# theteamatx/x-edr-trajectory-planning

Hardware: AMD Instinct MI355X
Metric: time-optimal path timings/s (7-DOF, 2000 s-samples), 1/2/4/8 MI355X + %HBM roofline (higher is better)
Workload: dtype f64

## Files before the change

### include/tpamd.h

```cpp
#ifndef TPAMD_H_
#define TPAMD_H_

#include <stddef.h>
#include <stdint.h>

#ifdef __cplusplus
extern "C" {
#endif

#define TPAMD_VERSION 200

#define TPAMD_E_INVALID_ARGUMENT (-1)
#define TPAMD_E_HIP (-2)
#define TPAMD_E_UNSUPPORTED (-3)
#define TPAMD_E_NO_DEVICE (-4)
#define TPAMD_E_STALE (-5)

#define TPAMD_PATH_OK 0
#define TPAMD_PATH_INFEASIBLE_BOUNDS 2
#define TPAMD_PATH_S_RANGE 3
#define TPAMD_PATH_SD_START_NEGATIVE 4
#define TPAMD_PATH_LOWER_GE_UPPER 5
#define TPAMD_PATH_TOO_FEW_SAMPLES 6
#define TPAMD_PATH_NO_CONNECTION 7
#define TPAMD_PATH_NAN_SD2 8
#define TPAMD_PATH_NONZERO_END 9
#define TPAMD_PATH_CRIT_INDEX_ZERO 10
#define TPAMD_PATH_NO_WAYPOINTS 11

typedef struct tpamd_engine tpamd_engine;

int tpamd_engine_create(int device_ordinal, tpamd_engine **out);
void tpamd_engine_destroy(tpamd_engine *engine);
int tpamd_version(void);
const char *tpamd_error_string(int code);
int tpamd_device_count(void);
int tpamd_engine_reserve(tpamd_engine *engine, int num_paths, int num_samples,
                         int num_rows);
int tpamd_engine_set_pipelining(tpamd_engine *engine, int mode);
int tpamd_engine_fence(tpamd_engine *engine, void *hip_stream);
size_t tpamd_engine_workspace_bytes(const tpamd_engine *engine);

typedef struct tpamd_joint_batch {
// ... 727 lines not shown
```

### x-edr-trajectory-planning_amd/csrc/tpamd_capi.hip

```cpp
#include "../../include/tpamd.h"

#include <hip/hip_runtime.h>

#include <algorithm>
#include <cmath>
#include <cstdio>
#include <cstdlib>
#include <cstring>
#include <mutex>
#include <new>
#include <vector>

#include "tpamd_kernels.h"
#include "tpamd_launch.h"
#include "tpamd_planner_set.h"
#include "tpamd_readout.h"
#include "tpamd_rescale.h"
#include "tpamd_buffer.h"
#include "tpamd_stop.h"
#include "tpamd_switch.h"
#include "tpamd_fit.h"
#include "tpamd_retarget.h"
#include "tpamd_pose_fit.h"
#include "tpamd_joint_fit.h"
// ... 488 lines not shown
    case TPAMD_E_INVALID_ARGUMENT: return "invalid argument";
    case TPAMD_E_HIP: return "HIP runtime error";
    case TPAMD_E_UNSUPPORTED: return "unsupported size";
    case TPAMD_E_NO_DEVICE: return "no HIP device";
    case TPAMD_E_STALE: return "engine state belongs to a different solve";
    case TPAMD_PATH_INFEASIBLE_BOUNDS: return "infeasible bounds: no upper > lower at a sample";
    case TPAMD_PATH_S_RANGE: return "s_start must be < s_end";
    case TPAMD_PATH_SD_START_NEGATIVE: return "sd_start must be >= 0";
    case TPAMD_PATH_LOWER_GE_UPPER: return "constraints must satisfy lower < upper";
    case TPAMD_PATH_TOO_FEW_SAMPLES: return "need at least 2 samples";
    case TPAMD_PATH_NO_CONNECTION: return "could not connect from critical point to initial trajectory portion";
    case TPAMD_PATH_NAN_SD2: return "no solution found (NaN in sd2)";
    case TPAMD_PATH_NONZERO_END: return "non-zero terminal velocity";
    case TPAMD_PATH_CRIT_INDEX_ZERO: return "critical point search degenerated to index 0";
    case TPAMD_PATH_NO_WAYPOINTS: return "path without waypoints";
    default: return "unknown";
  }
}

int tpamd_device_count(void) {
  int count = 0;
  if (hipGetDeviceCount(&count) != hipSuccess || count < 0) return 0;
  return count;
}

void tpamd_shard_bounds(int num_paths, int num_shards, int32_t *begin) {
  if (!begin || num_shards <= 0) return;
  const int total = num_paths > 0 ? num_paths : 0;
  const int base = total / num_shards, rem = total % num_shards;
  for (int r = 0; r <= num_shards; r++) begin[r] = r * base + (r < rem ? r : rem);
// ... 5261 lines not shown
```

### x-edr-trajectory-planning_amd/csrc/tpamd_sweep_joint.h

```cpp
#pragma once

#include <type_traits>

#include "tpamd_kernels.h"

namespace tpamd {

__device__ __forceinline__ double uniform_f64(double v) {
  const int lo = __builtin_amdgcn_readfirstlane(__double2loint(v));
  const int hi = __builtin_amdgcn_readfirstlane(__double2hiint(v));
  return __hiloint2double(hi, lo);
}
__device__ __forceinline__ double readlane_f64(double v, int lane) {
  const int lo = __builtin_amdgcn_readlane(__double2loint(v), lane);
  const int hi = __builtin_amdgcn_readlane(__double2hiint(v), lane);
  return __hiloint2double(hi, lo);
}
__device__ __forceinline__ int uniform_i32(int v) { return __builtin_amdgcn_readfirstlane(v); }
__device__ __forceinline__ int lds_word(const int *p) {
  return *(const volatile __attribute__((address_space(3))) int *)p;
}

template <int CTRL>
__device__ __forceinline__ double dpp_f64(double v) {
// ... 121 lines not shown
#define TPAMD_ACC(slot, var)
#endif
#else
#define TPAMD_T0(var)
#define TPAMD_ACC(slot, var)
#define TPAMD_T0C(var)
#define TPAMD_ACCC(slot, var)
#define TPAMD_CNT(slot)
#define TPAMD_ADD(slot, v)
#define TPAMD_CNTX(slot)
#endif

#ifndef TPAMD_CHAIN_GUESS
#define TPAMD_CHAIN_GUESS 0
#endif
constexpr int kTileSamples = 32;
template <int D>
struct TileCfg {
  static constexpr int kSamples = (D > 8) ? 16 : kTileSamples;
};

typedef double f64x2 __attribute__((ext_vector_type(2)));

template <int K>
struct RegPack {
  f64x2 v;
  RegPack<K - 1> rest;
  template <int LIMIT>
  __device__ __forceinline__ void load(const f64x2 *src, int c) {
    if (c < LIMIT) v = src[c];
    rest.template load<LIMIT>(src, c + 64);
  }
  template <int LIMIT>
  __device__ __forceinline__ void store(f64x2 *dst, int c) const {
    if (c < LIMIT) dst[c] = v;
    rest.template store<LIMIT>(dst, c + 64);
  }
};
template <>
struct RegPack<0> {
  template <int LIMIT> __device__ __forceinline__ void load(const f64x2 *, int) {}
  template <int LIMIT> __device__ __forceinline__ void store(f64x2 *, int) const {}
};

template <int D>
struct JointLayout {
  static constexpr int PARTS = (D <= 7) ? 4 : ((D <= 16) ? 2 : 1);
  static constexpr int RPL = (D + PARTS - 1) / PARTS;
  static constexpr int kCandLanes = 2 * D * PARTS;
  static constexpr int kRows16 = (kCandLanes + 15) / 16;
  static_assert(kCandLanes <= 64, "candidate lanes must fit one wave");
  static constexpr int kChain = 16;
  static constexpr int GRP = 64 / kChain;
  static constexpr int CPL = (2 * D + GRP - 1) / GRP;
  static constexpr int VPL = (D + GRP - 1) / GRP;
  static constexpr unsigned long long kPart0 =
      (GRP == 4) ? 0x1111111111111111ull : ((GRP == 2) ? 0x5555555555555555ull : ~0ull);
// ... 19 lines not shown
  mutable long long diagx[kDiagExt];
#endif
  int N, lane;
  double ds, two_ds;
  double *sd2;
  double *tiles;
  const uint8_t *typel;
  double *sdd_g;
  const double *m_g;
  const double *rec;
  int tag0, tag1;
  double *qd_g, *qdd_g;
  const double *aml;
  uint32_t *dirty;
  int end_idx;
  double lim;
  double chk_hi[L::RPL];
  double vel_hi;
  double vel_lo;
  int vel_mode;
  double ex_hi[E ? E : 1];
  int own_off;
  int chk_off[L::RPL];
  int vel_off;
  double row_lo, row_hi;
  double v_lim[L::CPL];
  int v_off[L::CPL];
  double vv_hi[L::VPL];
  double va_hi[L::VPL];
  int vv_off[L::VPL];

  struct Rows {
    f64x2 own;
    f64x2 chk[L::RPL];
    f64x2 vel;
  };

  static __device__ __forceinline__ void wave_lds_sync() {
    __builtin_amdgcn_fence(__ATOMIC_ACQ_REL, "wavefront");
    __builtin_amdgcn_wave_barrier();
  }

  struct Prefetch {
    RegPack<kChunksPerLane> r;
    double m;
    int tag;
  };
  __device__ __forceinline__ void issue_tile_loads(int t, Prefetch &pf) const {
    const f64x2 *src = reinterpret_cast<const f64x2 *>(rec + (size_t)t * kTile * R);
    pf.r.template load<kChunks>(src, lane);
    pf.m = m_g[min(t * kTile + (lane & (kTile - 1)), N - 1)];
    pf.tag = t;
  }
  __device__ __forceinline__ void store_tile(int slot, const Prefetch &pf) const {
    f64x2 *dst = reinterpret_cast<f64x2 *>(tiles + (size_t)slot * kTile * R);
    pf.r.template store<kChunks>(dst, lane);
    wave_lds_sync();
    if (lane < kTile) {
      const int i = min(pf.tag * kTile + lane, N - 1);
      f64x2 mt;
      mt.x = pf.m;
// ... 50 lines not shown
    if (QDD) {
      const double v2 = v * v;
      double acc = pr.x * a + pr.y * v2;
      if (acc < -amx) acc = -amx;
      if (acc > amx) acc = amx;
      qdd_g[o] = acc;
    }
  }
  __device__ __forceinline__ void emit_value(int i, int d, f64x2 pr, double v, double a,
                                             double amx) const {
    const size_t o = (size_t)i * D + d;
    if (qd_g) emit_pair<true, false>(o, pr, v, a, amx);
    if (qdd_g) emit_pair<false, true>(o, pr, v, a, amx);
  }
  __device__ __forceinline__ int emit_range(int lo, int hi, int wv, int nwv, const int *stop = nullptr,
                                            int stop_value = 0) const {
    if (qd_g != nullptr && qdd_g != nullptr) return emit_trips<true, true>(lo, hi, wv, nwv, stop, stop_value);
    if (qd_g != nullptr) return emit_trips<true, false>(lo, hi, wv, nwv, stop, stop_value);
    if (qdd_g != nullptr) return emit_trips<false, true>(lo, hi, wv, nwv, stop, stop_value);
    return hi + 1;
  }
  template <bool QD, bool QDD>
  __device__ __forceinline__ int emit_trips(int lo, int hi, int wv, int nwv, const int *stop,
                                            int stop_value) const {
    int s0 = lo + 64 * wv;
    if (hi < lo || s0 > hi) return hi + 1;
    if (stop != nullptr && uniform_i32(lds_word(stop)) == stop_value) return s0;
    const int step = 64 * nwv;
    const f64x2 *rec2 = reinterpret_cast<const f64x2 *>(rec);
    constexpr int G = (D <= 8) ? D : 5;
    constexpr int NG = (D + G - 1) / G;
    int ln = lane;
    asm volatile("" : "+v"(ln));
    int se0[D];
#pragma unroll
    for (int p = 0; p < D; p++) se0[p] = (64 * p + ln) / D;
    auto joint_of = [&](int p) { return 64 * p + ln - se0[p] * D; };
    f64x2 pr[2][G];
    double s2l[2], al[2];
    auto issue_sample = [&](int t0, int h) {
      const int mine = min(t0 + lane, hi);
      s2l[h] = sd2[mine];
// ... 33 lines not shown
          for (int g = 0; g < G; g++) {
            const int p = k * G + g;
            if (p >= D) continue;
            const int se = min(se0[p], last), dd = joint_of(p);
            const int src = se << 2;
            const double v = __hiloint2double(__builtin_amdgcn_ds_bpermute(src, __double2hiint(vl)),
                                              __builtin_amdgcn_ds_bpermute(src, __double2loint(vl)));
            const double a = __hiloint2double(__builtin_amdgcn_ds_bpermute(src, __double2hiint(al[h])),
                                              __builtin_amdgcn_ds_bpermute(src, __double2loint(al[h])));
            emit_pair<QD, QDD>((size_t)(s0 + se) * D + dd, pr[set][g], v, a, aml[dd]);
            if (p & 1) __builtin_amdgcn_sched_barrier(0);
          }
        }
        s0 = nxt;
        if (s0 > hi) return hi + 1;
        if (stop != nullptr && uniform_i32(lds_word(stop)) == stop_value) return s0;
      }
    }
  }
  __device__ __forceinline__ void mark_dirty(int i) const {
    if (lane == 0) atomicOr(&dirty[i >> 5], 1u << (i & 31));
  }

  template <bool MAX>
  __device__ __forceinline__ double find_sdd(const Rows &r, double s2, int &win) const {
    constexpr double kSentinel = MAX ? -DBL_MAX : DBL_MAX;
    bool vel_bad;
    if (E == 0) {
      const double vv = (r.vel.x * r.vel.x) * s2;
      vel_bad = (vv + kTiny < 0.0) | (vv - kTiny > vel_hi);
    } else {
// ... 125 lines not shown
  }

  struct Carry {
    int idx;
    double cur;
    double m_i;
    double m_n;
    double nxt;
    int t_i, t_n;
    int win;
  };
  static constexpr int kContinue = -2;

  template <bool FWD>
  __device__ __forceinline__ int extremal_step(Carry &c, const Rows &use, Rows &stage, Prefetch &pf,
                                               int idx_start, bool &pair_signal, bool &pair_wait) {
    constexpr int dir = FWD ? 1 : -1;
#define TPAMD_PAIR_SIGNAL()                                   \
  do {                                                        \
    if (pair_signal) {                                        \
      __threadfence_block();                                  \
      __syncthreads();                                        \
      pair_signal = false;                                    \
    }                                                         \
  } while (0)
#define TPAMD_PAIR_WAIT()                                     \
  do {                                                        \
    if (FWD && pair_wait) {                                   \
      __syncthreads();                                        \
      pair_wait = false;                                      \
    }                                                         \
  } while (0)
    const int idx = c.idx;
    const int nidx = idx + dir;
    const bool more = FWD ? (nidx < N - 2) : (nidx > 1);
    if (((nidx + dir) & (kTile - 1)) == (FWD ? 0 : kTile - 1))
      ensure_tile(nidx + dir, dir, pf);
    load_rows(nidx, stage);
    double m_nn;
    int t_nn;
    load_mt(nidx + dir, m_nn, t_nn);
    const double nxt_nn = sd2[nidx + dir];
    const double cur = c.cur, m_i = c.m_i, m_n = c.m_n, nxt = c.nxt;
    const bool on_boundary = is_tiny(cur - m_i);
    double sd2tmp, sddtmp;
    if (on_boundary && (c.t_i & kBndTrajectory) && (c.t_n & kBndTrajectory)) {
// ... 10 lines not shown
    if (!isnan(nxt) && (nxt < sd2tmp)) {
      TPAMD_PAIR_WAIT();
      sdd_at_intersection(idx);
      TPAMD_PAIR_SIGNAL();
      return FWD ? N - 1 : 0;
    }
    if (sd2tmp > m_n) {
      const double sdd_bound = FWD ? 0.5 * (m_n - cur) / ds : 0.5 * (cur - m_n) / ds;
      const bool deriv_invalid = !derivs_valid(idx, sdd_bound, FWD ? m_i : cur);
      const bool type_invalid = c.t_n & (FWD ? kBndSink : kBndSource);
      const bool stop = FWD ? (type_invalid || deriv_invalid)
                            : ((type_invalid || deriv_invalid) && !(idx_start != (N - 1)));
      if (stop) {
        end_idx = idx;
        TPAMD_PAIR_SIGNAL();
        TPAMD_PAIR_WAIT();
        return idx;
      }
      sd2tmp = m_n;
      sddtmp = sdd_bound;
      c.win = -1;
    }
    if (sd2tmp < 0) {
      TPAMD_PAIR_WAIT();
      c.win = -1;
      sd2tmp = 0.0;
      if (FWD) {
        if (idx <= 1) sddtmp = 0.0; else sddtmp = -sd2[idx - 1] / ds;
      } else {
        if (idx < N - 1) sddtmp = sd2[idx + 1] / ds; else sddtmp = 0.0;
      }
    }
    TPAMD_PAIR_WAIT();
    put_sd2(nidx, sd2tmp);
    put_sdd(idx, sddtmp);
    if (!more) end_idx = nidx;
    TPAMD_PAIR_SIGNAL();
    if (!more) return FWD ? N - 1 : 0;
    c.idx = nidx;
    c.cur = sd2tmp;
    c.m_i = m_n;
    c.t_i = c.t_n;
    c.m_n = uniform_f64(m_nn);
    c.t_n = uniform_i32(t_nn);
    c.nxt = uniform_f64(nxt_nn);
    return kContinue;
#undef TPAMD_PAIR_SIGNAL
#undef TPAMD_PAIR_WAIT
  }

// ... 8 lines not shown
    const int tj = max(j, 0) / kTile, tjn = max(jn, 0) / kTile;
    const bool resident = (tj == tag0 || tj == tag1) && (tjn == tag0 || tjn == tag1);
    if (in_loop && j >= 0 && j < N && resident) {
      const f64x2 mt_j = record(j)[kMt], mt_n = record(jn)[kMt];
      m_j = mt_j.x;
      m_jn = mt_n.x;
      const double nxt = sd2[jn];
      elig = (__double2loint(mt_j.y) & kBndTrajectory) && (__double2loint(mt_n.y) & kBndTrajectory) &&
             !(!isnan(nxt) && (nxt < m_jn)) && !(m_jn < 0);
    }
    const unsigned long long mask = __ballot(elig);
    const int L = (~mask == 0ull) ? 64 : (__ffsll((long long)~mask) - 1);
    if (L == 0) return 0;
    const double cur_k = (lane == 0) ? c.cur : m_j;
    const double sddv = FWD ? 0.5 * (m_jn - cur_k) / ds : 0.5 * (cur_k - m_jn) / ds;
    if (lane < L) {
      sd2[j + dir] = m_jn;
      sdd_g[j] = sddv;
    }
    wave_lds_sync();
    c.idx += dir * L;
    c.cur = readlane_f64(m_jn, L - 1);
    return L;
  }

  template <bool FWD>
  __device__ __forceinline__ int follow_chain(Carry &c, Prefetch &pf, int &next_win, bool &curve) {
    constexpr int dir = FWD ? 1 : -1;
    constexpr int K = L::kChain;
    next_win = -1;
    curve = false;
    const int wl = c.win;
    const int r = (wl / L::PARTS) >> 1;
// ... 96 lines not shown
    const int idx = c.idx, nidx = idx + dir;
    const bool more = FWD ? (nidx < N - 2) : (nidx > 1);
    const double cur = c.cur, m_n = c.m_n;
    const double sdd_bound = FWD ? 0.5 * (m_n - cur) / ds : 0.5 * (cur - m_n) / ds;
    const bool deriv_invalid = !derivs_valid(idx, sdd_bound, FWD ? c.m_i : cur);
    const bool type_invalid = c.t_n & (FWD ? kBndSink : kBndSource);
    const bool stop = FWD ? (type_invalid || deriv_invalid)
                          : ((type_invalid || deriv_invalid) && !(idx_start != (N - 1)));
    if (stop) {
      end_idx = idx;
      return idx;
    }
    double sd2tmp = m_n, sddtmp = sdd_bound;
    c.win = -1;
    if (sd2tmp < 0) {
      sd2tmp = 0.0;
      if (FWD) {
        if (idx <= 1) sddtmp = 0.0; else sddtmp = -sd2[idx - 1] / ds;
      } else {
        if (idx < N - 1) sddtmp = sd2[idx + 1] / ds; else sddtmp = 0.0;
      }
    }
    put_sd2(nidx, sd2tmp);
    put_sdd(idx, sddtmp);
    if (!more) {
      end_idx = nidx;
      return FWD ? N - 1 : 0;
    }
    c.idx = nidx;
    c.cur = sd2tmp;
// ... 15 lines not shown
    load_mt(idx, m0, t0);
    load_mt(idx + dir, m1, t1);
    c.m_i = uniform_f64(m0); c.m_n = uniform_f64(m1);
    c.t_i = uniform_i32(t0); c.t_n = uniform_i32(t1);
    c.nxt = uniform_f64(sd2[idx + dir]);
    c.win = -1;
    TPAMD_ACC(26, ti_);
  }

  template <bool FWD>
  __device__ __forceinline__ int add_extremal(int idx_start, Prefetch &pf, bool pair_signal = false,
                                              bool wait_pair = false) {
#define TPAMD_PAIR_SIGNAL()                                   \
  do {                                                        \
    if (pair_signal) {                                        \
      __threadfence_block();                                  \
      __syncthreads();                                        \
      pair_signal = false;                                    \
    }                                                         \
  } while (0)
    if (FWD ? !(idx_start < N - 2) : !(idx_start > 1)) {
      end_idx = idx_start;
      TPAMD_PAIR_SIGNAL();
      if (wait_pair) __syncthreads();
      return FWD ? N - 1 : 0;
    }
    Rows rows_a, rows_b;
    Carry c;
    init_carry<FWD>(idx_start, c, rows_a, pf, true);
    if (wait_pair && is_tiny(c.cur - c.m_i) && (c.t_i & kBndTrajectory) && (c.t_n & kBndTrajectory)) {
      __syncthreads();
      wait_pair = false;
    }
    bool trust = true;
    int last_win = -1;
    for (;;) {
#define TPAMD_TRY_FOLLOW()                                                                   \
  if (is_tiny(c.cur - c.m_i) && (c.t_i & kBndTrajectory) && (c.t_n & kBndTrajectory)) {      \
    TPAMD_T0(tfb_);                                                                          \
    const int run = uniform_i32(follow_boundary<FWD>(c));                                    \
    TPAMD_ACC(25, tfb_);                                                                     \
    if (run > 0) {                                                                           \
      TPAMD_CNT(8);                                                                          \
      TPAMD_PAIR_SIGNAL();                                                                   \
      if (FWD ? !(c.idx < N - 2) : !(c.idx > 1)) {                                           \
        end_idx = c.idx;                                                                     \
        return FWD ? N - 1 : 0;                                                              \
      }                                                                                      \
// ... 25 lines not shown
      total = 1;          \
    }                                                                                        \
    if (total > 0) {                                                                         \
      if (FWD ? !(c.idx < N - 2) : !(c.idx > 1)) {                                           \
        end_idx = c.idx;                                                                     \
        return FWD ? N - 1 : 0;                                                              \
      }                                                                                      \
      init_carry<FWD>(c.idx, c, rows_a, pf, false);                                          \
      continue;                                                                              \
    }                                                                                        \
  } else {                                                                                   \
    last_win = c.win;                                                                        \
  }
      TPAMD_TRY_FOLLOW();
      TPAMD_T0(ts1_);
      int r = extremal_step<FWD>(c, rows_a, rows_b, pf, idx_start, pair_signal, wait_pair);
      TPAMD_ACC(24, ts1_);
      if (r != kContinue) return r;
      TPAMD_TRY_CHAIN();
      if (is_tiny(c.cur - c.m_i) && (c.t_i & kBndTrajectory) && (c.t_n & kBndTrajectory)) {
        load_rows(c.idx, rows_a);
        continue;
      }
      TPAMD_T0(ts2_);
      r = extremal_step<FWD>(c, rows_b, rows_a, pf, idx_start, pair_signal, wait_pair);
      TPAMD_ACC(24, ts2_);
      if (r != kContinue) return r;
      TPAMD_TRY_CHAIN();
    }
#undef TPAMD_TRY_CHAIN
#undef TPAMD_TRY_FOLLOW
#undef TPAMD_PAIR_SIGNAL
  }

  __device__ __forceinline__ int next_critical_point(int idx_lo, int idx_hi, int zlast) const {
    int c0 = -1;
    for (int base = idx_lo + 1; base <= idx_hi && c0 < 0; base += 256) {
      uint8_t ty[4];
#pragma unroll
      for (int u = 0; u < 4; u++) ty[u] = typel[min(base + 64 * u + lane, N - 1)];
// ... 493 lines not shown
      }
      if (P.count + 64 > kRefitCap) P.template flush<true>(diag);
      P.append(refit, j, m, m_next);
    }
  }
  P.template flush<true>(diag);
  __threadfence_block();
  __syncthreads();
  TPAMD_ACCC(22, tp0);
}

template <int D, int E = 0>
struct SweepLds {
  static constexpr int R = 2 * D + E + 2;
  static constexpr int kRingDoubles = 2 * 2 * TileCfg<D>::kSamples * R;
  __host__ __device__ static constexpr int n2(int N) { return (N + 1) & ~1; }
  __host__ __device__ static constexpr int words(int N) { return ((N + 31) / 32 + 1) & ~1; }
  __host__ __device__ static constexpr int type_bytes(int N) { return ((N + 15) / 16) * 16; }
  __host__ __device__ static constexpr size_t bytes(int N) {
    return (size_t)n2(N) * 8 + (size_t)kRingDoubles * 8 + type_bytes(N) + 64 +
           2 * (size_t)words(N) * 4 + 16 * 8 + 32;
  }
};
template <int D, int E = 0>
__host__ __device__ inline size_t sweep_joint_lds_bytes(int N) {
  return SweepLds<D, E>::bytes(N);
}

constexpr int kSweepWavesPerEu = 2;
constexpr int kSweepWavesPerEuWide = 1;
template <int D, int E = 0>
__global__ void __launch_bounds__(128)
__attribute__((amdgpu_waves_per_eu((D > 8) ? kSweepWavesPerEuWide : kSweepWavesPerEu,
                                   (D > 8) ? kSweepWavesPerEuWide : kSweepWavesPerEu)))
k_sweep_joint(int stride, int max_loops, JointSource src, Workspace ws, double *t_out, double *s_out,
// ... 17 lines not shown
      if (dtmax_out) dtmax_out[b] = -1.0;
    }
    return;
  }
  JS S;
  S.N = N; S.lane = lane;
  S.ds = ws.ds[b];
  S.two_ds = 2.0 * S.ds;
  S.sd2 = lds;
  double *ring = lds + LL::n2(N);
  S.tiles = ring + (size_t)w * 2 * JS::kTile * JS::R;
  uint8_t *typel = reinterpret_cast<uint8_t *>(ring + LL::kRingDoubles);
  S.typel = typel;
  int *xchg = reinterpret_cast<int *>(typel + LL::type_bytes(N));
  const int nw = LL::words(N);
  uint32_t *dirty = reinterpret_cast<uint32_t *>(xchg + 16);
  uint32_t *zero = dirty + nw;
  double *aml = reinterpret_cast<double *>(zero + nw);
  double *red = aml + 16;
  S.dirty = dirty;
  S.aml = aml;
  S.sdd_g = sdd_out + pb;
  S.m_g = ws.m + pb;
  S.rec = src.q12 + pb * JS::R;
  S.qd_g = qd_out ? qd_out + pb * D : nullptr;
  S.qdd_g = qdd_out ? qdd_out + pb * D : nullptr;
  S.end_idx = 0;
  S.tag0 = -1; S.tag1 = -1;
  double *sd2 = S.sd2;
  const double sd_start = ws.sd_start[b];
#ifdef TPAMD_DIAG
  long long(&diag)[32] = S.diag;
  long long(&diagx)[kDiagExt] = S.diagx;
  for (int k = 0; k < 32; k++) diag[k] = 0;
  for (int k = 0; k < kDiagExt; k++) diagx[k] = 0;
  volatile long long *fw_stamp = reinterpret_cast<volatile long long *>(red + 2);
#define TPAMD_DIAG_PTR S.diag
#else
#define TPAMD_DIAG_PTR nullptr
#endif
  boundary_passes_for_path<D, E>(src, ws, b, N, stride, tid, reinterpret_cast<uint8_t *>(sd2),
                           reinterpret_cast<uint8_t *>(sd2) + LL::type_bytes(N),
                           reinterpret_cast<char *>(ring), typel, (ws.keep_boundary & 1) != 0,
                           TPAMD_DIAG_PTR);
  constexpr int C = 2 * D + E;
  const double *lim_lo = src.lim + (size_t)b * 2 * C, *lim_hi = lim_lo + C;
  {
    typedef JointLayout<D> L;
    const double kInf = __longlong_as_double(0x7ff0000000000000LL);
    const bool is_cand = lane < L::kCandLanes;
    const int c = is_cand ? lane / L::PARTS : 0;
// ... 45 lines not shown
      S.vv_off[i] = has ? row : 0;
      S.vv_hi[i] = has ? lim_hi[D + row] : kInf;
      S.va_hi[i] = has ? lim_hi[row] : kInf;
    }
  }

  for (int i = tid; i < N; i += 128) {
    sd2[i] = qnan();
    S.sdd_g[i] = qnan();
  }
  for (int i = tid; i < 2 * nw; i += 128) dirty[i] = 0u;
  if (tid < D) aml[tid] = ws.amax ? ws.amax[(size_t)b * D + tid] : 0.0;
  __syncthreads();
  if (tid == 0) {
    xchg[2] = 0;
    xchg[6] = 0;
    sd2[0] = sd_start * sd_start;
    sd2[N - 1] = 0;
  }
  __syncthreads();

  int status = 0;
  int iforw_lo = 0, iback_hi = N - 1, iback_lo, iforw_hi, icrit, icrit_lo, icrit_hi;
  typename JS::Prefetch pf;
  pf.tag = -1;
  TPAMD_T0C(t_all);
  int emitted_hi = 0, upper_lo = N;
  bool first_pair_in_order = false;
  if (w == 0) {
    const int r = S.template add_extremal<false>(iback_hi, pf);
    if (lane == 0) { xchg[0] = r; xchg[7] = S.end_idx; }
// ... 36 lines not shown
    __syncthreads();
  }
  iback_lo = uniform_i32(xchg[0]);
  iforw_hi = uniform_i32(xchg[1]);
  TPAMD_ACCC(9, t_all);
  icrit_hi = iback_lo;
  if ((iforw_hi < icrit_hi) && ((icrit_hi < N - 2) && (icrit_hi >= 2))) {
    if (w == 0) S.put_sd2(icrit_hi, qnan());
    icrit_hi++;
    iback_lo++;
  }
  icrit_lo = iforw_hi;
  const int zlast = uniform_i32(S.last_flagged_below(icrit_hi));
  const double *m_g = ws.m + pb;
  if (max_loops <= 0) max_loops = max(100, 10 * N);
  double *crit_m = reinterpret_cast<double *>(xchg + 10);
  auto post_next_critical_point = [&](int lo) {
    TPAMD_T0(t0);
    int ic = uniform_i32(S.next_critical_point(lo, icrit_hi, zlast));
    TPAMD_ACC(2, t0);
#if defined(TPAMD_DIAG) && !defined(TPAMD_DIAG_LIGHT)
    {
      TPAMD_T0(tl_);
      if (ic != S.next_critical_point_literal(lo, icrit_hi)) TPAMD_CNT(7);
      TPAMD_ACC(18, tl_);
    }
#endif
    if (ic < 0 || ic >= N) ic = (int)(0.5 * (lo + icrit_hi));
    const double mc = m_g[min(max(ic, 0), N - 1)], mp = m_g[min(max(ic - 1, 0), N - 1)];
    if (ic >= 1) {
      const int ts = ic / JS::kTile;
      const int tag = (ts & 1) ? S.tag1 : S.tag0;
      if (tag != ts && pf.tag != ts) S.issue_tile_loads(ts, pf);
    }
    if (lane == 0) {
      xchg[9] = ic;
      crit_m[0] = mc;
      crit_m[1] = mp;
    }
  };
  __syncthreads();
  if (w == 1 && iforw_hi < icrit_hi) post_next_critical_point(icrit_lo);
  __threadfence_block();
  __syncthreads();
  for (int loop = 0; loop < max_loops; loop++) {
    if (iforw_hi >= icrit_hi) break;
    TPAMD_CNT(11);
#ifdef TPAMD_DIAG
    int bw_case = 2;
    long long bw_left = 0;
#endif
    icrit = uniform_i32(xchg[9]);
    const double m_c = uniform_f64(crit_m[0]), m_p = uniform_f64(crit_m[1]);
    if (w == 0 && icrit >= 1) {
      const int ts = (icrit - 1) / JS::kTile;
      const int tag = (ts & 1) ? S.tag1 : S.tag0;
      if (tag != ts && pf.tag != ts) S.issue_tile_loads(ts, pf);
    }
    if (icrit > 0 && icrit < N - 1 && w == 0) S.put_sd2(icrit, m_c);
    if (icrit < 1) { status = 10; break; }
    if (m_p <= m_c) {
      iback_hi = icrit - 1;
      if (w == 0) S.put_sd2(icrit - 1, m_p);
    } else {
      iback_hi = icrit;
    }
    iforw_lo = icrit;
    __syncthreads();
    {
      TPAMD_T0C(t0);
      if (w == 0) {
        const int r = S.template add_extremal<false>(iback_hi, pf, true);
        if (lane == 0) xchg[0] = r;
#ifdef TPAMD_DIAG
        const bool fw_was_done = lds_word(xchg + 6) == loop + 1;
#endif
        TPAMD_T0C(te);
        emitted_hi = uniform_i32(S.emit_range(max(min(S.end_idx - 1, emitted_hi), 0), icrit - 1,
                                              0, 1, xchg + 6, loop + 1));
        TPAMD_ACCC(12, te);
#ifdef TPAMD_DIAG
        bw_case = fw_was_done ? 0 : (lds_word(xchg + 6) == loop + 1) ? 1 : 2;
        bw_left = tpamd_stamp();
#endif
      } else {
        const int r = S.template add_extremal<true>(iforw_lo, pf, false, true);
#ifdef TPAMD_DIAG
        { const long long t = tpamd_stamp(); if (lane == 0) fw_stamp[0] = t; }
#endif
        if (lane == 0) {
          xchg[1] = r;
          *reinterpret_cast<volatile int *>(xchg + 6) = loop + 1;
        }
        if (r < icrit_hi) post_next_critical_point(r);
#ifdef TPAMD_DIAG
        { const long long t = tpamd_stamp(); if (lane == 0) fw_stamp[1] = t; }
#endif
      }
      TPAMD_ACCC(0, t0);
    }
    {
      TPAMD_T0C(t0);
      __threadfence_block();
#ifdef TPAMD_DIAG
      const long long fenced = tpamd_stamp();
#endif
      __syncthreads();
      TPAMD_ACCC(1, t0);
#ifdef TPAMD_DIAG
      if (w == 0) {
        const long long fw_done = fw_stamp[0], fw_at_c = fw_stamp[1];
        const long long fw_wait = (fenced > fw_at_c) ? fenced - fw_at_c : 0;
        diagx[0] += bw_case == 0;
        diagx[1] += bw_case == 1;
        diagx[2] += bw_case == 2;
        diagx[7] += fenced - t0;
        if (bw_case == 1) {
          diagx[3] += bw_left - fw_done;
          diagx[4] += fenced - t0;
          diagx[5] += fw_wait;
        } else if (bw_case == 0) {
          diagx[6] += fw_wait;
        }
      }
#endif
    }
    iback_lo = uniform_i32(xchg[0]);
    iforw_hi = uniform_i32(xchg[1]);
    if (iback_lo > icrit_lo) { status = 7; break; }
    icrit_lo = iforw_hi;
  }
  TPAMD_ACCC(5, t_all);
  if (lane == 0) {
    if (w == 0) { xchg[4] = emitted_hi; xchg[5] = upper_lo; }
    else xchg[3] = S.end_idx;
  }
  __threadfence_block();
  __syncthreads();

  TPAMD_T0C(t_tail);
  const double ds = S.ds;
  double *sdd = S.sdd_g;
  {
    int has_nan = 0;
    if (status == 0)
      for (int idx = tid; idx < N; idx += 128)
        if (isnan(sd2[idx])) has_nan = 1;
    if (has_nan) xchg[2] = 1;
    __syncthreads();
    if (status == 0 && xchg[2] != 0) status = 8;
  }
  if (status == 0) {
    for (int base = 0; base < N; base += 512) {
// ... 250 lines not shown
```

### x-edr-trajectory-planning_amd/engine.py

```python
import ctypes as C
import os

import numpy as np

from . import abi as _abi
from .abi import (
    ABI_SYMBOLS, DIAG_SO, HIPCC_FLAGS, MULTI_SO, PLAN_DEVICE_INFO_FIELDS, PLAN_RESOURCE_EXHAUSTED,
    PLANNER_CHECK_DTYPE, PLANNER_STATE_INFO_DTYPE, PLANNER_SUMMARY_DTYPE, REFINE_NO_SLOT, REFINE_NOTHING,
    REFINE_TOO_LONG, SWEEP_INSTANCES, TpamdError, _CartesianBatch, _CartesianInputs, _CheckOutputs,
    _FastestStopArgs, _JointBatch, _JointInputs, _PathOutputs, _PlanDeviceInfo, _PlannerCheck, _PlannerSetConfig,
    _RefineOptions, _RefineOutputs, _ResampleArgs, _RowsBatch, _RowsInputs, _Solution, _StopTrajectoryArgs,
    _WaypointBatch, _WaypointFitOutputs, _WaypointInputs, _ptr)

_SO = os.environ.get("TPAMD_LIBRARY") or os.path.join(_abi._CSRC, "libtpamd.so")

PATH_STATUS = {
    0: "ok", 2: "infeasible_bounds", 3: "s_range", 4: "sd_start_negative",
    5: "lower_ge_upper", 6: "too_few_samples", 7: "no_connection", 8: "nan_sd2",
    9: "nonzero_end", 10: "crit_index_zero", 11: "no_waypoints",
}

KERNEL_SWEEP = 4

_CARTESIAN_INPUT_KEYS = _CartesianInputs._keys_


def build_library(force=False, verbose=False, extra_flags=(), output=None):
    global _SO
    if output is not None:
        _SO = output
    return _abi._compile(_SO, extra_flags, force, verbose)


def build_multi_library(force=False, verbose=False):
# ... 1526 lines not shown
```

Measured before the change: 2.161 million.

## Decouple forward and backward sweep waves with an LDS work queue

The per-loop __syncthreads lockstep between the forward wave and the backward wave is replaced by a 4-entry LDS ring queue. The forward wave finds critical points, posts them, and keeps integrating ahead while the backward wave consumes entries and emits outputs. The first overlapping write is handed off through a compare-exchange in LDS, so neither wave has to block on a workgroup barrier. This is meant to remove barrier stalls and let the two directions overlap across loops. In exchange it adds spin-polling with s_sleep, a bounded-wait error status, and ordering logic that is subtle and could race.

```diff
diff --git a/include/tpamd.h b/include/tpamd.h
--- a/include/tpamd.h
+++ b/include/tpamd.h
@@ -27,6 +27,7 @@
 #define TPAMD_PATH_NONZERO_END 9
 #define TPAMD_PATH_CRIT_INDEX_ZERO 10
 #define TPAMD_PATH_NO_WAYPOINTS 11
+#define TPAMD_PATH_SWEEP_POLL_EXPIRED 12
 
 typedef struct tpamd_engine tpamd_engine;
 
diff --git a/x-edr-trajectory-planning_amd/csrc/tpamd_capi.hip b/x-edr-trajectory-planning_amd/csrc/tpamd_capi.hip
--- a/x-edr-trajectory-planning_amd/csrc/tpamd_capi.hip
+++ b/x-edr-trajectory-planning_amd/csrc/tpamd_capi.hip
@@ -526,6 +526,7 @@
     case TPAMD_PATH_NONZERO_END: return "non-zero terminal velocity";
     case TPAMD_PATH_CRIT_INDEX_ZERO: return "critical point search degenerated to index 0";
     case TPAMD_PATH_NO_WAYPOINTS: return "path without waypoints";
+    case TPAMD_PATH_SWEEP_POLL_EXPIRED: return "internal error: a bounded wait inside the sweep kernel ran out";
     default: return "unknown";
   }
 }
diff --git a/x-edr-trajectory-planning_amd/csrc/tpamd_sweep_joint.h b/x-edr-trajectory-planning_amd/csrc/tpamd_sweep_joint.h
--- a/x-edr-trajectory-planning_amd/csrc/tpamd_sweep_joint.h
+++ b/x-edr-trajectory-planning_amd/csrc/tpamd_sweep_joint.h
@@ -159,6 +159,20 @@
 #ifndef TPAMD_CHAIN_GUESS
 #define TPAMD_CHAIN_GUESS 0
 #endif
+constexpr int kQRing = 4;
+constexpr int kQEntryWords = 16;
+constexpr int kQPosted = 6;
+constexpr int kQDone1 = 9;
+constexpr int kQAbort = 10;
+constexpr int kQStatus = 11;
+constexpr int kQPollErr = 12;
+constexpr int kQeState = 0, kQeCrit = 1, kQeBackHi = 2, kQeCritLo = 3, kQeKind = 4;
+constexpr int kQeDeferred = 8;
+constexpr int kQKindLoop = 0, kQKindEnd = 1, kQKindCritZero = 2;
+constexpr int kQPollBound = 1 << 22;
+constexpr int kStatusSweepPoll = 12;
+static_assert(kQPosted < 16 && kQPollErr < 16 && kQeDeferred + 4 <= kQEntryWords, "loop queue layout");
+
 constexpr int kTileSamples = 32;
 template <int D>
 struct TileCfg {
@@ -181,11 +195,16 @@
     if (c < LIMIT) dst[c] = v;
     rest.template store<LIMIT>(dst, c + 64);
   }
+  __device__ __forceinline__ void drop() {
+    v = f64x2{0.0, 0.0};
+    rest.drop();
+  }
 };
 template <>
 struct RegPack<0> {
   template <int LIMIT> __device__ __forceinline__ void load(const f64x2 *, int) {}
   template <int LIMIT> __device__ __forceinline__ void store(f64x2 *, int) const {}
+  __device__ __forceinline__ void drop() {}
 };
 
 template <int D>
@@ -235,6 +254,10 @@
   const double *aml;
   uint32_t *dirty;
   int end_idx;
+  int *qc, *qe;
+  int qn;
+  int pair_mode;
+  bool fw_first;
   double lim;
   double chk_hi[L::RPL];
   double vel_hi;
@@ -262,10 +285,97 @@
     __builtin_amdgcn_wave_barrier();
   }
 
+  static __device__ __forceinline__ void lds_store(int *p, int v) {
+    *(volatile __attribute__((address_space(3))) int *)p = v;
+  }
+  template <int CAUSE>
+  __device__ __forceinline__ bool q_wait(int word, int value) const {
+    if (uniform_i32(lds_word(qc + word)) >= value) return true;
+#ifdef TPAMD_DIAG
+    const long long tw_ = tpamd_stamp();
+#endif
+    bool ok = false;
+    for (int n = 0;; n++) {
+      __builtin_amdgcn_s_sleep(1);
+      if (uniform_i32(lds_word(qc + word)) >= value) { ok = true; break; }
+      if (uniform_i32(lds_word(qc + kQAbort)) != 0) break;
+      if (n >= kQPollBound) {
+        if (lane == 0) { lds_store(qc + kQPollErr, 1); lds_store(qc + kQAbort, 1); }
+        break;
+      }
+    }
+#ifdef TPAMD_DIAG
+    diagx[CAUSE] += tpamd_stamp() - tw_;
+    diagx[CAUSE + 9] += 1;
+#endif
+    return ok;
+  }
+  __device__ __forceinline__ void pair_release() {
+    __threadfence_block();
+    int old = 0;
+    if (lane == 0) {
+      int expected = 4 * qn + 1;
+      __hip_atomic_compare_exchange_strong(qe + kQeState, &expected, 4 * qn + 2, __ATOMIC_RELAXED,
+                                           __ATOMIC_RELAXED, __HIP_MEMORY_SCOPE_WORKGROUP);
+      old = expected;
+    }
+    fw_first = uniform_i32(old) == 4 * qn + 3;
+    __threadfence_block();
+#ifdef TPAMD_DIAG
+    diagx[5] += fw_first;
+    diagx[6] += !fw_first;
+#endif
+    if (fw_first && lane == 0) {
+      const int c = lds_word(qe + kQeCrit);
+      const volatile __attribute__((address_space(3))) double *pd =
+          (const volatile __attribute__((address_space(3))) double *)(qe + kQeDeferred);
+      sd2[c + 1] = pd[0];
+      sdd_g[c] = pd[1];
+    }
+    __threadfence_block();
+    if (lane == 0) lds_store(qc + kQDone1, qn + 1);
+  }
+  __device__ __forceinline__ bool pair_defer(double v, double a) {
+    if (uniform_i32(lds_word(qc + kQDone1)) > qn) { pair_mode = 0; return false; }
+    int old = 0;
+    if (lane == 0) {
+      volatile __attribute__((address_space(3))) double *pd =
+          (volatile __attribute__((address_space(3))) double *)(qe + kQeDeferred);
+      pd[0] = v;
+      pd[1] = a;
+    }
+    __threadfence_block();
+    if (lane == 0) {
+      int expected = 4 * qn + 1;
+      __hip_atomic_compare_exchange_strong(qe + kQeState, &expected, 4 * qn + 3, __ATOMIC_RELAXED,
+                                           __ATOMIC_RELAXED, __HIP_MEMORY_SCOPE_WORKGROUP);
+      old = expected;
+    }
+    old = uniform_i32(old);
+    if (old == 4 * qn + 1) {
+      TPAMD_CNTX(5);
+      pair_mode = 2;
+      return true;
+    }
+    __threadfence_block();
+    pair_mode = 0;
+    return false;
+  }
+  template <int CAUSE>
+  __device__ __forceinline__ void pair_settle() {
+    q_wait<CAUSE>(kQDone1, qn + 1);
+    pair_mode = 0;
+  }
+
   struct Prefetch {
     RegPack<kChunksPerLane> r;
     double m;
     int tag;
+    __device__ __forceinline__ void drop() {
+      r.drop();
+      m = 0.0;
+      tag = -1;
+    }
   };
   __device__ __forceinline__ void issue_tile_loads(int t, Prefetch &pf) const {
     const f64x2 *src = reinterpret_cast<const f64x2 *>(rec + (size_t)t * kTile * R);
@@ -346,18 +456,18 @@
     if (qdd_g) emit_pair<false, true>(o, pr, v, a, amx);
   }
   __device__ __forceinline__ int emit_range(int lo, int hi, int wv, int nwv, const int *stop = nullptr,
-                                            int stop_value = 0) const {
-    if (qd_g != nullptr && qdd_g != nullptr) return emit_trips<true, true>(lo, hi, wv, nwv, stop, stop_value);
-    if (qd_g != nullptr) return emit_trips<true, false>(lo, hi, wv, nwv, stop, stop_value);
-    if (qdd_g != nullptr) return emit_trips<false, true>(lo, hi, wv, nwv, stop, stop_value);
+                                            int go_value = 0) const {
+    if (qd_g != nullptr && qdd_g != nullptr) return emit_trips<true, true>(lo, hi, wv, nwv, stop, go_value);
+    if (qd_g != nullptr) return emit_trips<true, false>(lo, hi, wv, nwv, stop, go_value);
+    if (qdd_g != nullptr) return emit_trips<false, true>(lo, hi, wv, nwv, stop, go_value);
     return hi + 1;
   }
   template <bool QD, bool QDD>
   __device__ __forceinline__ int emit_trips(int lo, int hi, int wv, int nwv, const int *stop,
-                                            int stop_value) const {
+                                            int go_value) const {
     int s0 = lo + 64 * wv;
     if (hi < lo || s0 > hi) return hi + 1;
-    if (stop != nullptr && uniform_i32(lds_word(stop)) == stop_value) return s0;
+    if (stop != nullptr && uniform_i32(lds_word(stop)) != go_value) return s0;
     const int step = 64 * nwv;
     const f64x2 *rec2 = reinterpret_cast<const f64x2 *>(rec);
     constexpr int G = (D <= 8) ? D : 5;
@@ -421,7 +531,7 @@
         }
         s0 = nxt;
         if (s0 > hi) return hi + 1;
-        if (stop != nullptr && uniform_i32(lds_word(stop)) == stop_value) return s0;
+        if (stop != nullptr && uniform_i32(lds_word(stop)) != go_value) return s0;
       }
     }
   }
@@ -577,22 +687,18 @@
 
   template <bool FWD>
   __device__ __forceinline__ int extremal_step(Carry &c, const Rows &use, Rows &stage, Prefetch &pf,
-                                               int idx_start, bool &pair_signal, bool &pair_wait) {
+                                               int idx_start, bool &pair_signal) {
     constexpr int dir = FWD ? 1 : -1;
 #define TPAMD_PAIR_SIGNAL()                                   \
   do {                                                        \
     if (pair_signal) {                                        \
-      __threadfence_block();                                  \
-      __syncthreads();                                        \
+      pair_release();                                         \
       pair_signal = false;                                    \
     }                                                         \
   } while (0)
 #define TPAMD_PAIR_WAIT()                                     \
   do {                                                        \
-    if (FWD && pair_wait) {                                   \
-      __syncthreads();                                        \
-      pair_wait = false;                                      \
-    }                                                         \
+    if (FWD && pair_mode != 0) pair_settle<0>();              \
   } while (0)
     const int idx = c.idx;
     const int nidx = idx + dir;
@@ -633,7 +739,6 @@
       if (stop) {
         end_idx = idx;
         TPAMD_PAIR_SIGNAL();
-        TPAMD_PAIR_WAIT();
         return idx;
       }
       sd2tmp = m_n;
@@ -650,9 +755,10 @@
         if (idx < N - 1) sddtmp = sd2[idx + 1] / ds; else sddtmp = 0.0;
       }
     }
-    TPAMD_PAIR_WAIT();
-    put_sd2(nidx, sd2tmp);
-    put_sdd(idx, sddtmp);
+    if (!(FWD && pair_mode == 1 && pair_defer(sd2tmp, sddtmp))) {
+      put_sd2(nidx, sd2tmp);
+      put_sdd(idx, sddtmp);
+    }
     if (!more) end_idx = nidx;
     TPAMD_PAIR_SIGNAL();
     if (!more) return FWD ? N - 1 : 0;
@@ -691,9 +797,18 @@
     if (L == 0) return 0;
     const double cur_k = (lane == 0) ? c.cur : m_j;
     const double sddv = FWD ? 0.5 * (m_jn - cur_k) / ds : 0.5 * (cur_k - m_jn) / ds;
-    if (lane < L) {
+    const bool first = FWD && pair_mode == 1;
+    if (lane < L && !(first && lane == 0)) {
       sd2[j + dir] = m_jn;
       sdd_g[j] = sddv;
+    }
+    if (first) {
+      if (pair_defer(readlane_f64(m_jn, 0), readlane_f64(sddv, 0))) {
+        TPAMD_CNTX(6);
+      } else if (lane == 0) {
+        sd2[j + dir] = m_jn;
+        sdd_g[j] = sddv;
+      }
     }
     wave_lds_sync();
     c.idx += dir * L;
@@ -820,6 +935,7 @@
     double sd2tmp = m_n, sddtmp = sdd_bound;
     c.win = -1;
     if (sd2tmp < 0) {
+      if (FWD && pair_mode != 0) pair_settle<0>();
       sd2tmp = 0.0;
       if (FWD) {
         if (idx <= 1) sddtmp = 0.0; else sddtmp = -sd2[idx - 1] / ds;
@@ -865,24 +981,19 @@
 #define TPAMD_PAIR_SIGNAL()                                   \
   do {                                                        \
     if (pair_signal) {                                        \
-      __threadfence_block();                                  \
-      __syncthreads();                                        \
+      pair_release();                                         \
       pair_signal = false;                                    \
     }                                                         \
   } while (0)
+    pair_mode = (FWD && wait_pair) ? 1 : 0;
     if (FWD ? !(idx_start < N - 2) : !(idx_start > 1)) {
       end_idx = idx_start;
       TPAMD_PAIR_SIGNAL();
-      if (wait_pair) __syncthreads();
       return FWD ? N - 1 : 0;
     }
     Rows rows_a, rows_b;
     Carry c;
     init_carry<FWD>(idx_start, c, rows_a, pf, true);
-    if (wait_pair && is_tiny(c.cur - c.m_i) && (c.t_i & kBndTrajectory) && (c.t_n & kBndTrajectory)) {
-      __syncthreads();
-      wait_pair = false;
-    }
     bool trust = true;
     int last_win = -1;
     for (;;) {
@@ -938,7 +1049,7 @@
   }
       TPAMD_TRY_FOLLOW();
       TPAMD_T0(ts1_);
-      int r = extremal_step<FWD>(c, rows_a, rows_b, pf, idx_start, pair_signal, wait_pair);
+      int r = extremal_step<FWD>(c, rows_a, rows_b, pf, idx_start, pair_signal);
       TPAMD_ACC(24, ts1_);
       if (r != kContinue) return r;
       TPAMD_TRY_CHAIN();
@@ -947,7 +1058,7 @@
         continue;
       }
       TPAMD_T0(ts2_);
-      r = extremal_step<FWD>(c, rows_b, rows_a, pf, idx_start, pair_signal, wait_pair);
+      r = extremal_step<FWD>(c, rows_b, rows_a, pf, idx_start, pair_signal);
       TPAMD_ACC(24, ts2_);
       if (r != kContinue) return r;
       TPAMD_TRY_CHAIN();
@@ -1471,11 +1582,12 @@
 struct SweepLds {
   static constexpr int R = 2 * D + E + 2;
   static constexpr int kRingDoubles = 2 * 2 * TileCfg<D>::kSamples * R;
+  static constexpr int kXchgWords = 16 + kQRing * kQEntryWords;
   __host__ __device__ static constexpr int n2(int N) { return (N + 1) & ~1; }
   __host__ __device__ static constexpr int words(int N) { return ((N + 31) / 32 + 1) & ~1; }
   __host__ __device__ static constexpr int type_bytes(int N) { return ((N + 15) / 16) * 16; }
   __host__ __device__ static constexpr size_t bytes(int N) {
-    return (size_t)n2(N) * 8 + (size_t)kRingDoubles * 8 + type_bytes(N) + 64 +
+    return (size_t)n2(N) * 8 + (size_t)kRingDoubles * 8 + type_bytes(N) + 4 * kXchgWords +
            2 * (size_t)words(N) * 4 + 16 * 8 + 32;
   }
 };
@@ -1523,7 +1635,7 @@
   S.typel = typel;
   int *xchg = reinterpret_cast<int *>(typel + LL::type_bytes(N));
   const int nw = LL::words(N);
-  uint32_t *dirty = reinterpret_cast<uint32_t *>(xchg + 16);
+  uint32_t *dirty = reinterpret_cast<uint32_t *>(xchg + LL::kXchgWords);
   uint32_t *zero = dirty + nw;
   double *aml = reinterpret_cast<double *>(zero + nw);
   double *red = aml + 16;
@@ -1536,6 +1648,8 @@
   S.qdd_g = qdd_out ? qdd_out + pb * D : nullptr;
   S.end_idx = 0;
   S.tag0 = -1; S.tag1 = -1;
+  S.qc = xchg; S.qe = xchg + 16; S.qn = 0;
+  S.pair_mode = 0; S.fw_first = false;
   double *sd2 = S.sd2;
   const double sd_start = ws.sd_start[b];
 #ifdef TPAMD_DIAG
@@ -1543,7 +1657,6 @@
   long long(&diagx)[kDiagExt] = S.diagx;
   for (int k = 0; k < 32; k++) diag[k] = 0;
   for (int k = 0; k < kDiagExt; k++) diagx[k] = 0;
-  volatile long long *fw_stamp = reinterpret_cast<volatile long long *>(red + 2);
 #define TPAMD_DIAG_PTR S.diag
 #else
 #define TPAMD_DIAG_PTR nullptr
@@ -1619,7 +1732,7 @@
   __syncthreads();
   if (tid == 0) {
     xchg[2] = 0;
-    xchg[6] = 0;
+    xchg[kQPosted] = 0; xchg[kQDone1] = 0; xchg[kQAbort] = 0; xchg[kQStatus] = 0; xchg[kQPollErr] = 0;
     sd2[0] = sd_start * sd_start;
     sd2[N - 1] = 0;
   }
@@ -1686,129 +1799,131 @@
   const int zlast = uniform_i32(S.last_flagged_below(icrit_hi));
   const double *m_g = ws.m + pb;
   if (max_loops <= 0) max_loops = max(100, 10 * N);
-  double *crit_m = reinterpret_cast<double *>(xchg + 10);
-  auto post_next_critical_point = [&](int lo) {
-    TPAMD_T0(t0);
-    int ic = uniform_i32(S.next_critical_point(lo, icrit_hi, zlast));
-    TPAMD_ACC(2, t0);
+  __syncthreads();
+  if (w == 1) {
+    int posted = 0, last_c = 0;
+    for (int loop = 0;; loop++) {
+      int kind = (loop >= max_loops || iforw_hi >= icrit_hi) ? kQKindEnd : kQKindLoop;
+      if (uniform_i32(lds_word(xchg + kQAbort)) != 0) break;
+      int ic = 0, bh = 0;
+      double mc = 0.0, mp = 0.0;
+      if (kind == kQKindLoop) {
+        TPAMD_CNT(11);
+        TPAMD_T0(t0);
+        ic = uniform_i32(S.next_critical_point(icrit_lo, icrit_hi, zlast));
+        TPAMD_ACC(2, t0);
 #if defined(TPAMD_DIAG) && !defined(TPAMD_DIAG_LIGHT)
-    {
-      TPAMD_T0(tl_);
-      if (ic != S.next_critical_point_literal(lo, icrit_hi)) TPAMD_CNT(7);
-      TPAMD_ACC(18, tl_);
-    }
+        {
+          TPAMD_T0(tl_);
+          if (ic != S.next_critical_point_literal(icrit_lo, icrit_hi)) TPAMD_CNT(7);
+          TPAMD_ACC(18, tl_);
+        }
 #endif
-    if (ic < 0 || ic >= N) ic = (int)(0.5 * (lo + icrit_hi));
-    const double mc = m_g[min(max(ic, 0), N - 1)], mp = m_g[min(max(ic - 1, 0), N - 1)];
-    if (ic >= 1) {
-      const int ts = ic / JS::kTile;
-      const int tag = (ts & 1) ? S.tag1 : S.tag0;
-      if (tag != ts && pf.tag != ts) S.issue_tile_loads(ts, pf);
+        if (ic < 0 || ic >= N) ic = (int)(0.5 * (icrit_lo + icrit_hi));
+        if (ic >= 1) {
+          const int ts = ic / JS::kTile;
+          const int tag = (ts & 1) ? S.tag1 : S.tag0;
+          if (tag != ts && pf.tag != ts) S.issue_tile_loads(ts, pf);
+        }
+        mc = uniform_f64(m_g[min(max(ic, 0), N - 1)]);
+        mp = uniform_f64(m_g[min(max(ic - 1, 0), N - 1)]);
+        if (ic < 1) kind = kQKindCritZero;
+        bh = (mp <= mc) ? ic - 1 : ic;
+      }
+      if (!S.template q_wait<2>(kQDone1, posted - (kQRing - 1))) break;
+      if (kind == kQKindLoop) {
+        if (posted > 0 && ic - 1 <= last_c + 1 && !S.template q_wait<1>(kQDone1, posted)) break;
+        if (ic < N - 1) S.put_sd2(ic, mc);
+        if (mp <= mc) S.put_sd2(ic - 1, mp);
+      }
+      int *q = xchg + 16 + kQEntryWords * (posted & (kQRing - 1));
+      if (lane == 0) {
+        q[kQeCrit] = ic;
+        q[kQeBackHi] = bh;
+        q[kQeCritLo] = icrit_lo;
+        q[kQeKind] = kind;
+      }
+      __threadfence_block();
+      if (lane == 0) {
+        JS::lds_store(q + kQeState, 4 * posted + 1);
+        JS::lds_store(xchg + kQPosted, posted + 1);
+      }
+      if (kind != kQKindLoop) break;
+      S.qe = q;
+      S.qn = posted;
+      posted++;
+      last_c = ic;
+      TPAMD_T0C(t0);
+      const int r = S.template add_extremal<true>(ic, pf, false, true);
+      TPAMD_ACCC(0, t0);
+      iforw_hi = r;
+      icrit_lo = r;
+    }
+    if (lane == 0) xchg[3] = S.end_idx;
+  } else {
+    int taken = 0;
+    for (;;) {
+      if (!S.template q_wait<0>(kQPosted, taken + 1)) break;
+      __threadfence_block();
+      int *q = xchg + 16 + kQEntryWords * (taken & (kQRing - 1));
+      const int kind = uniform_i32(lds_word(q + kQeKind));
+      if (kind != kQKindLoop) {
+        if (kind == kQKindCritZero) status = 10;
+        break;
+      }
+      TPAMD_CNT(11);
+      icrit = uniform_i32(lds_word(q + kQeCrit));
+      iback_hi = uniform_i32(lds_word(q + kQeBackHi));
+      icrit_lo = uniform_i32(lds_word(q + kQeCritLo));
+#ifdef TPAMD_DIAG
+      {
+        const int depth = uniform_i32(lds_word(xchg + kQPosted)) - taken;
+        diagx[1] += depth == 1;
+        diagx[2] += depth == 2;
+        diagx[3] += depth == 3;
+        diagx[4] += depth >= 4;
+      }
+#endif
+      {
+        const int ts = (icrit - 1) / JS::kTile;
+        const int tag = (ts & 1) ? S.tag1 : S.tag0;
+        if (tag != ts && pf.tag != ts) S.issue_tile_loads(ts, pf);
+      }
+      S.qe = q;
+      S.qn = taken;
+      TPAMD_T0C(t0);
+      const int r = S.template add_extremal<false>(iback_hi, pf, true);
+      TPAMD_ACCC(0, t0);
+      taken++;
+      iback_lo = r;
+      if (iback_lo > icrit_lo) { status = 7; break; }
+      TPAMD_T0C(te);
+      emitted_hi = uniform_i32(S.emit_range(max(min(S.end_idx - 1, emitted_hi), 0), icrit - 1,
+                                            0, 1, xchg + kQPosted, taken));
+      TPAMD_ACCC(12, te);
+      pf.drop();
     }
     if (lane == 0) {
-      xchg[9] = ic;
-      crit_m[0] = mc;
-      crit_m[1] = mp;
-    }
-  };
-  __syncthreads();
-  if (w == 1 && iforw_hi < icrit_hi) post_next_critical_point(icrit_lo);
-  __threadfence_block();
-  __syncthreads();
-  for (int loop = 0; loop < max_loops; loop++) {
-    if (iforw_hi >= icrit_hi) break;
-    TPAMD_CNT(11);
+      xchg[kQStatus] = status;
+      if (status != 0) JS::lds_store(xchg + kQAbort, 1);
+      xchg[4] = emitted_hi;
+      xchg[5] = upper_lo;
+    }
+  }
+  TPAMD_ACCC(5, t_all);
+  {
 #ifdef TPAMD_DIAG
-    int bw_case = 2;
-    long long bw_left = 0;
+    const long long tj_ = tpamd_stamp();
 #endif
-    icrit = uniform_i32(xchg[9]);
-    const double m_c = uniform_f64(crit_m[0]), m_p = uniform_f64(crit_m[1]);
-    if (w == 0 && icrit >= 1) {
-      const int ts = (icrit - 1) / JS::kTile;
-      const int tag = (ts & 1) ? S.tag1 : S.tag0;
-      if (tag != ts && pf.tag != ts) S.issue_tile_loads(ts, pf);
-    }
-    if (icrit > 0 && icrit < N - 1 && w == 0) S.put_sd2(icrit, m_c);
-    if (icrit < 1) { status = 10; break; }
-    if (m_p <= m_c) {
-      iback_hi = icrit - 1;
-      if (w == 0) S.put_sd2(icrit - 1, m_p);
-    } else {
-      iback_hi = icrit;
-    }
-    iforw_lo = icrit;
+    __threadfence_block();
     __syncthreads();
-    {
-      TPAMD_T0C(t0);
-      if (w == 0) {
-        const int r = S.template add_extremal<false>(iback_hi, pf, true);
-        if (lane == 0) xchg[0] = r;
 #ifdef TPAMD_DIAG
-        const bool fw_was_done = lds_word(xchg + 6) == loop + 1;
+    if (w == 1) diagx[4] += tpamd_stamp() - tj_;
+    else diagx[7] += tpamd_stamp() - tj_;
 #endif
-        TPAMD_T0C(te);
-        emitted_hi = uniform_i32(S.emit_range(max(min(S.end_idx - 1, emitted_hi), 0), icrit - 1,
-                                              0, 1, xchg + 6, loop + 1));
-        TPAMD_ACCC(12, te);
-#ifdef TPAMD_DIAG
-        bw_case = fw_was_done ? 0 : (lds_word(xchg + 6) == loop + 1) ? 1 : 2;
-        bw_left = tpamd_stamp();
-#endif
-      } else {
-        const int r = S.template add_extremal<true>(iforw_lo, pf, false, true);
-#ifdef TPAMD_DIAG
-        { const long long t = tpamd_stamp(); if (lane == 0) fw_stamp[0] = t; }
-#endif
-        if (lane == 0) {
-          xchg[1] = r;
-          *reinterpret_cast<volatile int *>(xchg + 6) = loop + 1;
-        }
-        if (r < icrit_hi) post_next_critical_point(r);
-#ifdef TPAMD_DIAG
-        { const long long t = tpamd_stamp(); if (lane == 0) fw_stamp[1] = t; }
-#endif
-      }
-      TPAMD_ACCC(0, t0);
-    }
-    {
-      TPAMD_T0C(t0);
-      __threadfence_block();
-#ifdef TPAMD_DIAG
-      const long long fenced = tpamd_stamp();
-#endif
-      __syncthreads();
-      TPAMD_ACCC(1, t0);
-#ifdef TPAMD_DIAG
-      if (w == 0) {
-        const long long fw_done = fw_stamp[0], fw_at_c = fw_stamp[1];
-        const long long fw_wait = (fenced > fw_at_c) ? fenced - fw_at_c : 0;
-        diagx[0] += bw_case == 0;
-        diagx[1] += bw_case == 1;
-        diagx[2] += bw_case == 2;
-        diagx[7] += fenced - t0;
-        if (bw_case == 1) {
-          diagx[3] += bw_left - fw_done;
-          diagx[4] += fenced - t0;
-          diagx[5] += fw_wait;
-        } else if (bw_case == 0) {
-          diagx[6] += fw_wait;
-        }
-      }
-#endif
-    }
-    iback_lo = uniform_i32(xchg[0]);
-    iforw_hi = uniform_i32(xchg[1]);
-    if (iback_lo > icrit_lo) { status = 7; break; }
-    icrit_lo = iforw_hi;
-  }
-  TPAMD_ACCC(5, t_all);
-  if (lane == 0) {
-    if (w == 0) { xchg[4] = emitted_hi; xchg[5] = upper_lo; }
-    else xchg[3] = S.end_idx;
-  }
-  __threadfence_block();
-  __syncthreads();
+  }
+  status = uniform_i32(xchg[kQStatus]);
+  if (uniform_i32(xchg[kQPollErr]) != 0) status = kStatusSweepPoll;
 
   TPAMD_T0C(t_tail);
   const double ds = S.ds;
diff --git a/x-edr-trajectory-planning_amd/engine.py b/x-edr-trajectory-planning_amd/engine.py
--- a/x-edr-trajectory-planning_amd/engine.py
+++ b/x-edr-trajectory-planning_amd/engine.py
@@ -17,7 +17,7 @@
 PATH_STATUS = {
     0: "ok", 2: "infeasible_bounds", 3: "s_range", 4: "sd_start_negative",
     5: "lower_ge_upper", 6: "too_few_samples", 7: "no_connection", 8: "nan_sd2",
-    9: "nonzero_end", 10: "crit_index_zero", 11: "no_waypoints",
+    9: "nonzero_end", 10: "crit_index_zero", 11: "no_waypoints", 12: "sweep_poll_expired",
 }
 
 KERNEL_SWEEP = 4
```

Result: faster. 2.220 million, median of 6 (+2.7%).
